# etri/bwa-mem-scale

Hardware: AMD Instinct MI355X
Metric: Mreads/sec through the GPU hot path (seed -> chain -> extend -> dedup, reads and index resident), 150bp SE vs a synthetic genome of GRCh38 size, at 1 MI355X; % HBM roofline in roofline.frac (higher is better)
Workload: dtype int64 intervals / int16 DP (two columns per register; int32 for queries beyond 191 bases or scores beyond 2^14)

## Files before the change

bwa-mem-scale_amd/bwams/capi.py:

```python
from __future__ import annotations

import ctypes as C
import os
import subprocess

import numpy as np

PKG = os.path.dirname(os.path.dirname(os.path.abspath(__file__)))
LIB_PATH = os.environ.get("BWAMS_LIB") or os.path.join(PKG, "_build", "libbwams.so")

SMEM_DTYPE = np.dtype([("rid", "<u4"), ("m", "<u4"), ("n", "<u4"), ("pad_", "<u4"),
                       ("k", "<i8"), ("l", "<i8"), ("s", "<i8")])
SEQPAIR_DTYPE = np.dtype([(n, "<i4") for n in
                          ("idr", "idq", "id", "len1", "len2", "h0", "seqid", "regid",
                           "score", "tle", "gtle", "qle", "gscore", "max_off")])

SYMBOLS = [
    "bwams_strerror", "bwams_last_error", "bwams_device_count", "bwams_debug_reload",
    "bwams_index_open", "bwams_index_from_host", "bwams_index_from_device", "bwams_index_close",
    "bwams_index_bytes", "bwams_index_build", "bwams_index_fetch", "bwams_index_save", "bwams_reg2aln_run", "bwams_reg2aln_run_sam", "bwams_reg2aln_fetch",
    "bwams_index_set_contig_names", "bwams_index_set_contig_annos", "bwams_sam_upload", "bwams_sam_run", "bwams_sam_run_pe", "bwams_sam_run_emf", "bwams_sam_fetch",
    "bwams_process_chunk", "bwams_process_chunk_smart", "bwams_process_chunk2", "bwams_emf_regs_merge", "bwams_fastq_decode", "bwams_fastq_info", "bwams_fastq_has_qual", "bwams_fastq_fetch", "bwams_fastq_to_batch", "bwams_fastq_to_batch_opt", "bwams_fastq_close", "bwams_batch_create", "bwams_batch_destroy", "bwams_seed_fmi",
    "bwams_seed_upload", "bwams_seed_run", "bwams_seed_counts", "bwams_seed_fetch",
    "bwams_ert_from_host", "bwams_ert_open", "bwams_ert_close", "bwams_ert_bytes", "bwams_ert_set_fat", "bwams_seed_run_ert",
    "bwams_ert_build", "bwams_ert_info", "bwams_ert_fetch", "bwams_ert_save", "bwams_debug_sort", "bwams_debug_regs_upload", "bwams_debug_aln_lists",
    "bwams_debug_ext_regs_upload", "bwams_debug_dedup_counts", "bwams_debug_pair_regs_upload", "bwams_debug_pair_counts", "bwams_debug_chain_counts", "bwams_debug_chain_lane_counts",
    "bwams_emf_build", "bwams_emf_info", "bwams_emf_table_fetch", "bwams_emf_save",
    "bwams_bsw_extend", "bwams_bsw_upload", "bwams_bsw_run", "bwams_bsw_fetch",
    "bwams_batch_stats", "bwams_batch_sync", "bwams_ksw_align",
    "bwams_index_build_fma", "bwams_index_set_fma", "bwams_index_fetch_fma",
    "bwams_index_from_fasta", "bwams_index_from_fasta_file", "bwams_index_load_bns",
    "bwams_emf_open", "bwams_emf_from_host", "bwams_emf_close", "bwams_emf_probe",
    "bwams_emf_from_device", "bwams_emf_run", "bwams_emf_fetch",
    "bwams_index_set_contigs", "bwams_chain_run", "bwams_chain_fetch", "bwams_chain_upload",
# ... 1297 lines not shown
        L.bwams_reg2aln_run.argtypes = [vp, vp, i32, vp, vp, vp]
        L.bwams_reg2aln_fetch.argtypes = [vp, vp, i64, vp, i64, vp, i64]
        L.bwams_debug_regs_upload.argtypes = [vp, vp, i64, vp, i64]
        L.bwams_debug_aln_lists.argtypes = [vp, vp]
        L.bwams_debug_ext_regs_upload.argtypes = [vp, vp, i64, vp, i64]
        L.bwams_debug_dedup_counts.argtypes = [vp, vp]
        L.bwams_debug_pair_regs_upload.argtypes = [vp, vp, i64, vp, i64]
        L.bwams_debug_pair_counts.argtypes = [vp, vp]
        L.bwams_debug_chain_counts.argtypes = [vp, vp]
        L.bwams_debug_chain_lane_counts.argtypes = [vp, vp]
        L.bwams_index_build_fma.argtypes = [vp, C.c_int, C.c_int]
        L.bwams_index_set_fma.argtypes = [vp, vp, C.c_int, vp, C.c_int]
        L.bwams_index_fetch_fma.argtypes = [vp, vp, vp]
        L.bwams_index_bytes.restype = i64
        L.bwams_index_bytes.argtypes = [vp]
        L.bwams_batch_create.argtypes = [vp, i64, i64, i64, i64, vp]
        L.bwams_batch_destroy.argtypes = [vp]
        L.bwams_seed_fmi.argtypes = [vp, vp, vp, vp, i64, vp, vp, i64, vp, vp, i64, vp, vp]
        L.bwams_seed_upload.argtypes = [vp, vp, vp, vp, i64]
        L.bwams_index_set_contigs.argtypes = [vp, vp, i32]
        L.bwams_chain_run.argtypes = [vp, vp, vp, vp]
        L.bwams_chain_fetch.argtypes = [vp, vp, i64, vp, i64, vp]
        L.bwams_chain_upload.argtypes = [vp, vp, i64, vp, i64, vp]
        L.bwams_extend_build.argtypes = [vp, vp, vp, vp]
        L.bwams_extend_run.argtypes = [vp, vp, vp]
        L.bwams_extend_fetch.argtypes = [vp, vp, i64, vp, vp]
        L.bwams_extend_tasks_fetch.argtypes = [vp, i32, vp, i64, vp, i64, vp, i64, vp, vp, vp]
        L.bwams_dedup_run.argtypes = [vp, vp, vp]
        L.bwams_dedup_fetch.argtypes = [vp, vp, i64, vp]
        L.bwams_pestat.argtypes = [vp, vp, vp]
# ... 199 lines not shown
            blob += (a if isinstance(a, bytes) else a.encode()) + b"\0"
        off.append(len(blob))
        off = np.asarray(off, np.int32)
        _chk(lib().bwams_index_set_contig_annos(self.h, bytes(blob), _p(off)), "bwams_index_set_contig_annos")

    def debug_sort(self, k, s, q, which: int, mode: int = 0):
        k = np.ascontiguousarray(k, np.int64); s = np.ascontiguousarray(s, np.int32); q = np.ascontiguousarray(q, np.int32)
        out = np.zeros(len(k), np.int32)
        _chk(lib().bwams_debug_sort(self.h, _p(k), _p(s), _p(q), len(k), which, mode, _p(out)), "bwams_debug_sort")
        return out

    @property
    def nbytes(self) -> int:
        return lib().bwams_index_bytes(self.h)

    def close(self):
        if self.h:
            lib().bwams_index_close(self.h)
            self.h = None


class Emf:

    def __init__(self, index: Index, table=None, path: str | None = None, device_table=None):
        self.index = index
        self.h = C.c_void_p()
        self._keep = device_table
        if device_table is not None:
            t = device_table
            _chk(lib().bwams_emf_from_device(index.h, t.seed_len, t.seq_len, t.loc_table.data_ptr(), t.loc_table.numel(),
                                             t.seed_table.data_ptr(), t.seed_table.shape[0], C.byref(self.h)),
                 "bwams_emf_from_device")
        elif path is not None:
            _chk(lib().bwams_emf_open(index.h, path.encode(), C.byref(self.h)), "bwams_emf_open")
# ... 921 lines not shown
```

bwa-mem-scale_amd/csrc/api.hip:

```cpp
#include <fcntl.h>
#include <sys/mman.h>
#include <sys/stat.h>
#include <unistd.h>

#include <algorithm>
#include <cstring>

#include "stage_state.h"

namespace bwams {

static Knobs g_knobs;
static std::once_flag g_knobs_once;
static int env_int(const char *name, int dflt) { const char *e = getenv(name); return e && *e ? atoi(e) : dflt; }
void knobs_reload() {
    Knobs k;
    { const char *vb = getenv("BWAMS_VERBOSE"); k.verbose = vb && *vb && *vb != '0'; }
    k.debug = env_int("BWAMS_DEBUG", 0);
    k.poison = env_int("BWAMS_POISON", 0);
    k.bwd_min_list = env_int("BWAMS_BWD_MIN_LIST", k.bwd_min_list); k.bwd_cols = env_int("BWAMS_BWD_COLS", k.bwd_cols);
    k.bwd_late_list = env_int("BWAMS_BWD_LATE_LIST", k.bwd_late_list);
    k.bwd_dry_min_list = env_int("BWAMS_BWD_DRY_MIN_LIST", k.bwd_dry_min_list); k.bwd_dry_cols = env_int("BWAMS_BWD_DRY_COLS", k.bwd_dry_cols);
    k.bwd_dry_late_list = env_int("BWAMS_BWD_DRY_LATE_LIST", k.bwd_dry_late_list);
    k.r3_beside = env_int("BWAMS_SEED_R3_BESIDE", 1);
    k.ext_max_rounds = env_int("BWAMS_EXT_MAX_ROUNDS", 0); k.ext_all_rounds = getenv("BWAMS_EXT_ALL_ROUNDS") != nullptr;
    k.ext_inplace = env_int("BWAMS_EXT_INPLACE", 1);
    k.dedup_seq = env_int("BWAMS_DEDUP_SEQ", 0) == 1;
    k.dedup_count = env_int("BWAMS_DEDUP_COUNT", 0) == 1;
    k.pair_count = env_int("BWAMS_PAIR_COUNT", 0) == 1;
    k.pair_drop_plan = getenv("BWAMS_PAIR_DROP_PLAN") != nullptr;
    k.trace_pair = env_int("BWAMS_TRACE_PAIR", 0);
    k.bsw_pk = env_int("BWAMS_BSW_PK", 1);
    k.chain_batch = env_int("BWAMS_CHAIN_BATCH", 1);
    k.chain_count = env_int("BWAMS_CHAIN_COUNT", 0) == 1;
    k.depth_combine = env_int("BWAMS_DEPTH_COMBINE", 1);
    k.pileup_tiled = env_int("BWAMS_PILEUP_TILED", 1);
    k.qc_lanes = env_int("BWAMS_QC_LANES", 1);
    k.recal_lds = env_int("BWAMS_RECAL_LDS", 1);
    k.ert_ticket = env_int("BWAMS_ERT_TICKET", 1); k.ert_grid = env_int("BWAMS_ERT_GRID", -1); k.ert_fat = env_int("BWAMS_ERT_FAT", 1);
    g_knobs = k;
}
const Knobs &knobs() {
    std::call_once(g_knobs_once, knobs_reload);
    return g_knobs;
}

static thread_local std::string g_last_error;
void set_last_error(const std::string &s) { g_last_error = s; }

int check_device(int device) {
    int n = 0;
    hipError_t e = hipGetDeviceCount(&n);
    if (e != hipSuccess || n <= 0) {
        set_last_error(std::string("no HIP device: ") + hipGetErrorString(e));
// ... 205 lines not shown
```

bwa-mem-scale_amd/csrc/api_index.hip:

```cpp
#include <cstring>

#include "fmi_kernels.h"

namespace bwams {
int fmi_build_device(bwams_index *ix, const uint8_t *d_fw, int64_t l_pac, int keep_ref, int64_t chunk_rows, int verbose,
                     bwams_build_stats_t *bs);
}

using namespace bwams;

extern "C" {

static int index_finish(bwams_index *ix, const bwams_fmi_desc_t *d, const void *cp, const void *ms, const void *ls, const void *ref) {
    ix->fmi.cp = reinterpret_cast<const uint4 *>(cp);
    ix->fmi.cp2 = nullptr;
    ix->fmi.sa_ms = reinterpret_cast<const int8_t *>(ms);
    ix->fmi.sa_ls = reinterpret_cast<const uint32_t *>(ls);
    ix->fmi.ref = reinterpret_cast<const uint8_t *>(ref);
    if (d->ref_seq_len >= ((int64_t)1 << 36)) {
        set_last_error("text longer than 2^36 rows is not supported by the 36-bit interval packing");
        return BWAMS_ERR_UNSUPPORTED;
    }
    for (int i = 0; i < 5; ++i) ix->fmi.count[i] = d->count[i];
    ix->fmi.sentinel = d->sentinel_index;
// ... 174 lines not shown
    if (rc == BWAMS_ERR_IO) set_last_error("write failed: " + path);
    if (!rc && ix->bns) rc = bns_save(ix, prefix);
    return rc;
}

int bwams_index_close(bwams_index_t *ix) {
    if (!ix) return BWAMS_OK;
    (void)hipSetDevice(ix->device);
    delete ix->bns;
    delete ix;
    return BWAMS_OK;
}

int64_t bwams_index_bytes(const bwams_index_t *ix) { return ix ? ix->bytes : 0; }


static int fma_alloc(bwams_index *ix, int all_bp, int last_bp) {
    if (all_bp < 2 || all_bp > 11 || last_bp < 2 || last_bp > 13) {
        set_last_error("FMA depths must be 2..11 (all_smem) and 2..13 (last_smem)");
        return BWAMS_ERR_ARG;
    }
    BWAMS_HIP(hipSetDevice(ix->device));
    ix->d_all.release();
    ix->d_last.release();
    ix->fmi.all_smem = nullptr;
    ix->fmi.last_smem = nullptr;
    BWAMS_HIP(ix->d_all.alloc(((size_t)1 << (2 * all_bp)) * 128));
    BWAMS_HIP(ix->d_last.alloc(((size_t)1 << (2 * last_bp)) * 16));
    return BWAMS_OK;
}
// ... 44 lines not shown
```

bwa-mem-scale_amd/csrc/api_seed.hip:

```cpp
#include <algorithm>
#include <cstring>
#include <mutex>

#include <rocprim/rocprim.hpp>

#include "fmi_kernels.h"
#include "ert_kernels.h"
#include "stage_state.h"

namespace bwams {

int alloc_smem_buffers(bwams_batch *b, int64_t max_smem) {
    b->sd.d_pool.release(); b->sd.d_sorted.release(); b->sd.d_keys.release(); b->sd.d_keys2.release(); b->sd.d_vals.release();
    b->sd.d_vals2.release(); b->sd.d_work2.release(); b->sd.d_sa_off.release(); b->sd.d_sa_cnt.release();
    b->max_smem = max_smem;
    b->pool_cap = b->max_smem + seed_pool_slack(b->cu_count);
    BWAMS_HIP(b->sd.d_pool.alloc((size_t)b->pool_cap * sizeof(bwams_smem_t)));
    BWAMS_HIP(b->sd.d_sorted.alloc((size_t)b->max_smem * sizeof(bwams_smem_t)));
    BWAMS_HIP(b->sd.d_keys.alloc((size_t)b->pool_cap * 8));
    BWAMS_HIP(b->sd.d_keys2.alloc((size_t)b->pool_cap * 8));
    BWAMS_HIP(b->sd.d_vals.alloc((size_t)b->pool_cap * 4));
    BWAMS_HIP(b->sd.d_vals2.alloc((size_t)b->pool_cap * 4));
    BWAMS_HIP(b->sd.d_work2.alloc((size_t)b->pool_cap * sizeof(Round2Work)));
    BWAMS_HIP(b->sd.d_sa_off.alloc((size_t)(b->max_smem + 1) * 8));
// ... 4 lines not shown
int alloc_seed_tmp(bwams_batch *b) {
    size_t t1 = 0, t2 = 0;
    (void)rocprim::radix_sort_pairs(nullptr, t1, b->sd.d_keys.p, b->sd.d_keys2.p, b->sd.d_vals.p, b->sd.d_vals2.p,
                              (size_t)b->max_smem, 0, 64, b->stream);
    (void)rocprim::exclusive_scan(nullptr, t2, b->sd.d_sa_cnt.p, b->sd.d_sa_off.p, (int64_t)0, (size_t)b->max_smem + 1,
                            rocprim::plus<int64_t>(), b->stream);
    BWAMS_HIP(b->d_tmp.alloc(std::max(t1, t2)));
    return BWAMS_OK;
}

namespace {

int sort_pool(bwams_batch *b, const char *who, int64_t n_keys, int64_t n, int64_t *sa_cnt, int max_occ) {
    bwams_batch::Seed &sd = b->sd;
    hipStream_t st = b->stream;
    launch_make_keys(sd.d_pool.p, n_keys, sd.d_keys.p, sd.d_vals.p, (uint32_t)b->nseq, st);
    int rid_bits = 1;
    while (((int64_t)1 << rid_bits) <= b->nseq) rid_bits++;
    if (int rc = with_tmp(b, who, [&](void *tmp, size_t &tb) {
            return rocprim::radix_sort_pairs(tmp, tb, sd.d_keys.p, sd.d_keys2.p, sd.d_vals.p, sd.d_vals2.p, (size_t)n_keys, 0, 32 + rid_bits, st);
        })) return rc;
    launch_gather_sorted(sd.d_pool.p, sd.d_vals2.p, n, sd.d_sorted.p, sa_cnt, max_occ, st);
    return BWAMS_OK;
}

void fm_lookup(bwams_batch *b, int64_t n) {
    bwams_batch::Seed &sd = b->sd;
    launch_sa_lookup(b->idx->fmi, sd.d_sorted.p, n, sd.d_sa_off.p, sd.d_sa_coord.p, b->max_sa, sd.last_opt.max_occ, b->d_ctr.p, b->cu_count, b->stream);
}
void ert_locate(bwams_batch *b, int64_t n) {
    bwams_batch::Seed &sd = b->sd;
    launch_ert_locate(sd.ert->t, b->d_enc.p, b->d_cum.p, sd.d_sorted.p, n, sd.with_sa ? sd.d_sa_cnt.p : nullptr, sd.last_opt.max_occ, b->d_ctr.p,
                      sd.d_ert_stk.p, sd.ert_stk_frames, b->cu_count, b->stream);
}
int ert_gather(bwams_batch *b, int64_t n) {
    bwams_batch::Seed &sd = b->sd;
    const int64_t cap = n + n / 4 + 1024;
    BWAMS_HIP(sd.d_ert_redo.ensure((size_t)((n + 31) / 32) * 4, (size_t)((cap + 31) / 32) * 4));
    launch_ert_gather(sd.ert->t, sd.d_sorted.p, n, sd.d_sa_off.p, sd.d_sa_coord.p, b->max_sa, sd.last_opt.max_occ, b->d_ctr.p, sd.d_ert_stk.p,
                      sd.ert_stk_frames, sd.d_ert_redo.p, b->max_sa, b->cu_count, b->stream);
    return BWAMS_OK;
}

// ... 86 lines not shown
    b->sd.n_smem = b->sd.n_sa = 0;

    const uint4 *cp2 = nullptr;
    {
        bwams_index *ix = b->idx;
        std::lock_guard<std::mutex> lock(ix->cp2_mu);
        if (!ix->d_cp2.p) {
            DevBuf<> t;
            BWAMS_HIP(t.alloc(cp2_bytes(ix->n_blk)));
            launch_cp2_build(ix->fmi.cp, ix->n_blk, t.as<uint4>(), st);
            BWAMS_HIP(hipStreamSynchronize(st));
            ix->d_cp2 = std::move(t);
        }
        cp2 = ix->d_cp2.as<const uint4>();
    }
    SeedLaunch a;
    a.fmi = b->idx->fmi;
    a.fmi.cp2 = cp2;
    a.enc = b->d_enc.p;
    a.cum = b->d_cum.p;
    a.skip = b->has_skip ? b->d_skip.p : nullptr;
    a.nseq = b->nseq;
    a.packed = b->sd.d_packed.p;
    a.read_w = b->sd.read_w;
    a.read_cw = b->sd.read_cw;
    a.reads_in_lds = b->sd.read_w <= 40;
    a.debug = knobs().debug;
    a.min_seed_len = opt->min_seed_len;
    a.pool = b->sd.d_pool.p;
    a.pool_cap = b->pool_cap;
// ... 277 lines not shown
```

bwa-mem-scale_amd/csrc/common.h:

```cpp
#pragma once

#include <cstdlib>
#include <hip/hip_runtime.h>
#include <mutex>
#include <stdint.h>
#include <stdio.h>
#include <string>
#include <vector>

#include "../../include/bwams.h"
#include "stage_valid.h"

namespace bwams {

void set_last_error(const std::string &s);

struct Knobs {
    int verbose = 0;
    int debug = 0;
    int poison = 0;
    int bwd_min_list = 40, bwd_cols = 24, bwd_late_list = 8;
    int bwd_dry_min_list = 24, bwd_dry_cols = 8, bwd_dry_late_list = 12;
    int r3_beside = 1;
    int ext_max_rounds = 0;
    int ext_all_rounds = 0;
    int ext_inplace = 1;
    int dedup_seq = 0;
    int dedup_count = 0;
    int pair_count = 0;
    int pair_drop_plan = 0;
    int trace_pair = 0;
    int bsw_pk = 1;
    int chain_count = 0;
    int chain_batch = 1;
    int ert_fat = 1;
    int depth_combine = 1;
    int pileup_tiled = 1;
    int qc_lanes = 1;
    int recal_lds = 1;
    int ert_grid = -1, ert_ticket = 1;
};
const Knobs &knobs();
void knobs_reload();

template <class T> static inline hipError_t dev_malloc(T **p, size_t bytes) {
    const bool poison = knobs().poison != 0;
    hipError_t e = hipMalloc(reinterpret_cast<void **>(p), bytes);
    if (e == hipSuccess && poison && bytes) {
        e = hipMemset(*p, 0xAB, bytes);
        if (e == hipSuccess) e = hipDeviceSynchronize();
    }
    return e;
}

template <class T = void, bool Host = false> struct Buf {
    T *p = nullptr;
    size_t cap = 0;
    Buf() = default;
    Buf(Buf &&o) noexcept : p(o.p), cap(o.cap) { o.p = nullptr; o.cap = 0; }
    Buf &operator=(Buf &&o) noexcept {
        if (this != &o) { release(); p = o.p; cap = o.cap; o.p = nullptr; o.cap = 0; }
        return *this;
    }
    ~Buf() { release(); }
    template <class U> U *as() const { return reinterpret_cast<U *>(p); }
    void release() {
        if (p) (void)(Host ? hipHostFree(p) : hipFree(p));
        p = nullptr;
        cap = 0;
    }
    hipError_t alloc(size_t bytes) {
        release();
        hipError_t e = Host ? hipHostMalloc(&p, bytes, hipHostMallocDefault) : dev_malloc(&p, bytes);
        cap = p ? bytes : 0;
        return e;
    }
    hipError_t ensure(size_t bytes, size_t new_cap) { return bytes <= cap ? hipSuccess : alloc(new_cap); }
    hipError_t ensure(size_t bytes) { return ensure(bytes, bytes + bytes / 8 + 4096); }
    hipError_t ensure_n(size_t n) { return ensure(n * sizeof(T)); }
};
template <class T = void> using DevBuf = Buf<T, false>;
template <class T = void> using HostBuf = Buf<T, true>;

#define BWAMS_HIP(call)                                                                  \
    do {                                                                                 \
        hipError_t e_ = (call);                                                          \
        if (e_ != hipSuccess) {                                                          \
            char buf_[512];                                                              \
// ... 539 lines not shown
};
namespace bwams {
int fastq_classify(bwams_fastq *f, std::vector<uint8_t> *which);
int fastq_subset(bwams_fastq *f, const std::vector<int64_t> &ids, bwams_fastq **out);
int fastq_interleave(bwams_fastq *f1, bwams_fastq *f2, bwams_fastq **out);
}

struct bwams_index {
    int device = 0;
    bwams::DevFmi fmi{};
    int64_t bytes = 0;
    int64_t n_blk = 0, n_sa = 0;
    bwams::DevBuf<> d_cp, d_ms, d_ls, d_ref;
    bwams::DevBuf<> d_cp2;
    std::mutex cp2_mu;
    bwams::DevBuf<> d_all, d_last;
    bwams::DevBuf<> d_contigs;
    int32_t n_seqs = 0;
    bwams::DevBuf<> d_ctg_annos, d_ctg_anno_off;
    bwams::DevBuf<> d_ctg_names, d_ctg_off;
    bwams::BnsMeta *bns = nullptr;
    std::vector<std::string> h_ctg_names;
    bwams::DevBuf<> d_ctg_sorted;
    bool ctg_dup = false;
};

namespace bwams {
int bns_save(bwams_index *ix, const char *prefix);
int bam_names_index(bwams_index *ix, const char *names, const int32_t *name_off, int32_t n);
}

struct bwams_ert {
    bwams_index *idx = nullptr;
    bwams::DevErt t{};
    bwams::DevBuf<> d_kmer, d_mlt, d_cnt, d_fat;
    int64_t bytes = 0, mlt_bytes = 0, n_big = 0;
    float build_ms[3] = {0, 0, 0};
};

struct bwams_emf {
    bwams_index *idx = nullptr;
    bwams::DevEmf t{};
    bwams::DevBuf<> d_seeds, d_loc;
// ... 129 lines not shown
```

bwa-mem-scale_amd/csrc/fmi_kernels.h:

```cpp
#pragma once
#include "common.h"

namespace bwams {

struct SeedLaunch {
    DevFmi fmi;
    const uint8_t *enc;
    const int64_t *cum;
    const uint8_t *skip;
    const uint32_t *packed;
    int read_w, read_cw;
    int reads_in_lds;
    int debug;
    int64_t nseq;
    int min_seed_len;
    bwams_smem_t *pool;
    int64_t pool_cap;
    DevCounters *ctr;
    uint4 *prev;
    int prev_cap;
    int64_t prev_threads;
    BwdItem *bwd_items, *bwd_items_s;
    uint4 *bwd_ent;
    int64_t bwd_items_cap, bwd_ent_cap;
// ... 7 lines not shown
int64_t seed_pool_slack(int cu_count);

void launch_pack_reads(const uint8_t *enc, const int64_t *cum, int64_t nseq, int W, int cw, uint32_t *packed,
                       hipStream_t st);
void launch_mark(DevCounters *ctr, int which, hipStream_t st);
void launch_smem_round1(const SeedLaunch &a, int cu_count, hipStream_t st);
void launch_round2_work(const SeedLaunch &a, Round2Work *work, int64_t work_cap, int split_len,
                        int split_width, int cu_count, hipStream_t st);
void launch_smem_round2(const SeedLaunch &a, const Round2Work *work, int cu_count, hipStream_t st);
void launch_smem_bwd_wave(const SeedLaunch &a, int cu_count, hipStream_t st);
void launch_smem_round3(const SeedLaunch &a, int max_intv, int cu_count, hipStream_t st);

void launch_build_fma(const DevFmi &f, int all_bp, uint32_t *all_tab, int last_bp, uint4 *last_tab, hipStream_t st);

void launch_make_keys(const bwams_smem_t *pool, int64_t n, uint64_t *keys, uint32_t *vals, uint32_t hole_key_rid,
                      hipStream_t st);
void launch_gather_sorted(const bwams_smem_t *pool, const uint32_t *order, int64_t n, bwams_smem_t *sorted,
                          int64_t *sa_cnt, int max_occ, hipStream_t st);
void launch_sa_lookup(const DevFmi &f, const bwams_smem_t *sorted, int64_t n_smem, const int64_t *sa_off,
                      int64_t *coord, int64_t coord_cap, int max_occ, DevCounters *ctr, int cu_count,
                      hipStream_t st);

size_t cp2_bytes(int64_t n_blk);
void launch_cp2_build(const uint4 *cp, int64_t n_blk, uint4 *cp2, hipStream_t st);

}
```

bwa-mem-scale_amd/csrc/fmi_sal.hip:

```cpp
#include "fmi_kernels.h"

namespace bwams {
namespace {

__device__ __forceinline__ uint64_t mk64(uint32_t lo, uint32_t hi) {
    return (uint64_t)lo | ((uint64_t)hi << 32);
}

__global__ __launch_bounds__(256) void sa_lookup_kernel(DevFmi f, const bwams_smem_t *__restrict__ sm,
                                                        int64_t n_smem, const int64_t *__restrict__ sa_off,
                                                        int64_t *__restrict__ coord, int64_t coord_cap,
                                                        int max_occ, DevCounters *ctr) {
    const int64_t total = sa_off[n_smem] < coord_cap ? sa_off[n_smem] : coord_cap;
    unsigned long long lf = 0;
    __shared__ int64_t win_s[4][65];
    int64_t *const win = win_s[threadIdx.x >> 6];
    const int lane = (int)(threadIdx.x & 63);
    const int64_t n_waves = (int64_t)gridDim.x * 4, wave = (int64_t)blockIdx.x * 4 + (threadIdx.x >> 6);
    const int64_t per = ((total + n_waves - 1) / n_waves + 63) & ~(int64_t)63;
    const int64_t start = wave * per, end = start + per < total ? start + per : total;
    int64_t lo0 = 0;
    if (start < end) {
        int64_t a = 0, b = n_smem;
        while (b - a > 1) {
            const int64_t mid = (a + b) >> 1;
            if (sa_off[mid] <= start) a = mid; else b = mid;
        }
// ... 19 lines not shown
                const int64_t mid = (a + b) >> 1;
                if (sa_off[mid] <= g) a = mid; else b = mid;
            }
            lo = a;
        }
        {
            const int last = (int)((end - g0 < 64 ? end - g0 : 64) - 1);
            const uint32_t l_lo = (uint32_t)lo, l_hi = (uint32_t)((uint64_t)lo >> 32);
            lo0 = (int64_t)(((uint64_t)(uint32_t)__builtin_amdgcn_readlane((int)l_hi, last) << 32) | (uint32_t)__builtin_amdgcn_readlane((int)l_lo, last));
        }
        __builtin_amdgcn_wave_barrier();
        if (g >= end) continue;
        const int64_t k = sm[lo].k, s = sm[lo].s;
        const int64_t step = s > (int64_t)max_occ ? s / max_occ : 1;
        int64_t sp = k + (g - sa_off[lo]) * step;
        int64_t off = 0, val = 0;
        while (true) {
            if ((sp & 7) == 0) {
                val = ((int64_t)f.sa_ms[sp >> 3] << 32) + (int64_t)f.sa_ls[sp >> 3] + off;
                break;
            }
            const uint4 *p = f.cp + ((sp >> 6) << 2);
            const uint4 c01 = p[0], c23 = p[1], h01 = p[2], h23 = p[3];
            const int sh = 63 - (int)(sp & 63);
            const uint64_t h0 = mk64(h01.x, h01.y), h1 = mk64(h01.z, h01.w);
            const uint64_t h2 = mk64(h23.x, h23.y), h3 = mk64(h23.z, h23.w);
            int b = 4;
            uint64_t hb = 0;
            if ((h0 >> sh) & 1) { b = 0; hb = h0; }
            else if ((h1 >> sh) & 1) { b = 1; hb = h1; }
            else if ((h2 >> sh) & 1) { b = 2; hb = h2; }
            else if ((h3 >> sh) & 1) { b = 3; hb = h3; }
            if (b == 4) { val = 0; break; }
            const int y = (int)(sp & 63);
            const uint64_t mask = y ? (~0ull << (64 - y)) : 0ull;
            const int64_t cnt = (int64_t)(b == 0 ? mk64(c01.x, c01.y) : b == 1 ? mk64(c01.z, c01.w) : b == 2 ? mk64(c23.x, c23.y) : mk64(c23.z, c23.w));
            sp = (b == 0 ? f.count[0] : b == 1 ? f.count[1] : b == 2 ? f.count[2] : f.count[3]) + cnt +
                 __popcll(hb & mask);
            off++;
            lf++;
        }
        coord[g] = val;
    }
    for (int o = 32; o > 0; o >>= 1)
        lf += mk64(__shfl_down((uint32_t)lf, o), __shfl_down((uint32_t)(lf >> 32), o));
    if ((threadIdx.x & 63) == 0 && lf) atomicAdd(&ctr->n_lf_steps, lf);
    if (blockIdx.x == 0 && threadIdx.x == 0) ctr->n_sa_lookups = (unsigned long long)sa_off[n_smem];
}

}

void launch_sa_lookup(const DevFmi &f, const bwams_smem_t *sorted, int64_t n_smem, const int64_t *sa_off,
                      int64_t *coord, int64_t coord_cap, int max_occ, DevCounters *ctr, int cu_count,
                      hipStream_t st) {
    if (n_smem <= 0) return;
    sa_lookup_kernel<<<cu_count * 8, 256, 0, st>>>(f, sorted, n_smem, sa_off, coord, coord_cap, max_occ, ctr);
}

}
```

bwa-mem-scale_amd/csrc/fmi_seed.hip:

```cpp
#include "fmi_kernels.h"
#include "wave_ops.h"

namespace bwams {

namespace {

constexpr int kBlock = 256;
constexpr int kBlocksPerCU = 6;

__device__ __forceinline__ uint64_t mk64(uint32_t lo, uint32_t hi) {
    return (uint64_t)lo | ((uint64_t)hi << 32);
}

struct Occ4 {
    int64_t v[4];
};

template <int CTRL>
__device__ __forceinline__ uint32_t qdpp(uint32_t v) {
    return (uint32_t)__builtin_amdgcn_update_dpp(0, (int)v, CTRL, 0xF, 0xF, false);
}

__device__ __forceinline__ void occ_from_block(const uint4 &c01, const uint4 &c23, const uint4 &h01,
                                               const uint4 &h23, int64_t pos, Occ4 &o) {
// ... 1246 lines not shown
                em_n = (uint32_t)j;
                em_k = ck; em_l = cl; em_s = cs;
                x = next_x;
                phase = PH_PIVOT;
            }
            j++;
        }
        if (phase == PH_HOLD) phase = PH_FWD;
        wave_emit(a, wo, em, rid, em_m, em_n, em_k, em_l, em_s);
    }
    wave_emit_finish(a, wo, true);
    flush_counters(a.ctr, n_ext, n_blk, true);
}

__global__ void make_keys_kernel(const bwams_smem_t *pool, int64_t n, uint64_t *keys, uint32_t *vals,
                                 uint32_t hole_key_rid) {
    const int64_t i = (int64_t)blockIdx.x * blockDim.x + threadIdx.x;
    if (i < n) {
        const bwams_smem_t s = pool[i];
        const uint32_t rid = s.rid == kHoleRid ? hole_key_rid : s.rid;
        keys[i] = ((uint64_t)rid << 32) | ((uint64_t)(s.m & 0xffff) << 16) | (uint64_t)(s.n & 0xffff);
        vals[i] = (uint32_t)i;
    }
}

__global__ void gather_sorted_kernel(const bwams_smem_t *pool, const uint32_t *order, int64_t n,
                                     bwams_smem_t *sorted, int64_t *sa_cnt, int max_occ) {
    const int64_t i = (int64_t)blockIdx.x * blockDim.x + threadIdx.x;
    if (i < n) {
        const bwams_smem_t s = pool[order[i]];
        sorted[i] = s;
        if (sa_cnt) sa_cnt[i] = s.s < (int64_t)max_occ ? s.s : (int64_t)max_occ;
    }
}

__global__ void cpi_build_kernel(const uint4 *__restrict__ cp, int64_t n_blk, uint4 *__restrict__ out) {
// ... 60 lines not shown
void launch_smem_round2(const SeedLaunch &a, const Round2Work *work, int cu_count, hipStream_t st) {
    smem_search_kernel<false><<<grid_for(a.nseq, cu_count), kBlock, lds_bytes_search(a), st>>>(a, work);
}

void launch_smem_bwd_wave(const SeedLaunch &a, int cu_count, hipStream_t st) {
    if (a.bwd_min_list <= 0) return;
    const size_t lds = (size_t)(kBlock / 64) * (kBwdMaxList * 16 + 16 * (size_t)(a.read_w <= kBwdReadLds ? a.read_w : 0));
    smem_bwd_kernel<<<cu_count * 8, kBlock, lds, st>>>(a);
}

void launch_smem_round3(const SeedLaunch &a, int max_intv, int cu_count, hipStream_t st) {
    seed_strategy_kernel<<<grid_for(a.nseq, cu_count), kBlock, lds_bytes(a), st>>>(a, max_intv);
}

void launch_make_keys(const bwams_smem_t *pool, int64_t n, uint64_t *keys, uint32_t *vals, uint32_t hole_key_rid,
                      hipStream_t st) {
    if (n <= 0) return;
    make_keys_kernel<<<(unsigned)((n + 255) / 256), 256, 0, st>>>(pool, n, keys, vals, hole_key_rid);
}

void launch_gather_sorted(const bwams_smem_t *pool, const uint32_t *order, int64_t n, bwams_smem_t *sorted,
                          int64_t *sa_cnt, int max_occ, hipStream_t st) {
    if (n <= 0) return;
    gather_sorted_kernel<<<(unsigned)((n + 255) / 256), 256, 0, st>>>(pool, order, n, sorted, sa_cnt, max_occ);
}

}
```

include/bwams.h:

```cpp
#ifndef BWAMS_H
#define BWAMS_H

#include <stddef.h>
#include <stdint.h>
#include "bwams_types.h"

#ifdef __cplusplus
extern "C" {
#endif

#define BWAMS_OK               0
#define BWAMS_ERR_DEVICE      -1
#define BWAMS_ERR_IO          -2
#define BWAMS_ERR_ARG         -3
#define BWAMS_ERR_CAPACITY    -4
#define BWAMS_ERR_NOMEM       -5
#define BWAMS_ERR_UNSUPPORTED -6

typedef struct bwams_index bwams_index_t;
typedef struct bwams_batch bwams_batch_t;
typedef struct bwams_emf bwams_emf_t;

const char *bwams_strerror(int code);
const char *bwams_last_error(void);
// ... 69 lines not shown
typedef struct bwams_deflater bwams_deflater_t;
typedef struct bwams_deflate_stats {
    int64_t members, in_bytes, out_bytes;
    float ms_upload, ms_kernel, ms_download;
} bwams_deflate_stats_t;
#define BWAMS_DEFLATE_EOF 0x1
int64_t bwams_deflate_bound(int64_t n_bytes);
int bwams_deflater_create(int device, int64_t max_in_bytes, bwams_deflater_t **out);
int bwams_deflater_run(bwams_deflater_t *d, const void *in, int64_t n_bytes, int in_on_device, void *out, int64_t out_cap,
                       int out_on_device, int32_t flags, int64_t *n_out, bwams_deflate_stats_t *stats);
int bwams_deflater_destroy(bwams_deflater_t *d);
int bwams_index_load_bns(bwams_index_t *idx, const char *prefix);

int bwams_index_close(bwams_index_t *idx);
int64_t bwams_index_bytes(const bwams_index_t *idx);


int bwams_batch_create(bwams_index_t *idx, int64_t max_reads, int64_t max_bases,
                       int64_t max_smem, int64_t max_sa, bwams_batch_t **out);
int bwams_batch_destroy(bwams_batch_t *b);


int bwams_seed_fmi(bwams_batch_t *b,
                   const uint8_t *enc_qdb, const int64_t *cum_len, const uint8_t *skip,
                   int64_t nseq, const bwams_seed_opt_t *opt,
                   bwams_smem_t *smem_out, int64_t smem_cap, int64_t *n_smem,
                   int64_t *sa_coord, int64_t sa_cap, int64_t *sa_off, int64_t *n_sa);

int bwams_seed_upload(bwams_batch_t *b, const uint8_t *enc_qdb, const int64_t *cum_len,
                      const uint8_t *skip, int64_t nseq);
// ... 411 lines not shown
```

Baseline: 11.25.

## Add lazily built dense suffix-array table and narrow seed sort keys

Builds a full-resolution (stride 1 by default) suffix-array coordinate table on the device the first time seeding with SA lookup runs. sa_lookup then does one indexed load instead of walking the BWT up to seven LF steps per hit to reach a sampled SA entry. The table is about 8 bytes per reference position (tens of GB for a GRCh38-sized genome). It can be refused under a byte cap or released when another allocation runs out of memory. Separately, seed sort keys use 8-bit position fields when reads are at most 255 bases, cutting radix sort passes.

```diff
diff --git a/bwa-mem-scale_amd/bwams/capi.py b/bwa-mem-scale_amd/bwams/capi.py
--- a/bwa-mem-scale_amd/bwams/capi.py
+++ b/bwa-mem-scale_amd/bwams/capi.py
@@ -18,6 +18,7 @@
 SYMBOLS = [
     "bwams_strerror", "bwams_last_error", "bwams_device_count", "bwams_debug_reload",
     "bwams_index_open", "bwams_index_from_host", "bwams_index_from_device", "bwams_index_close",
+    "bwams_debug_sa_dense_state", "bwams_debug_sa_dense_fetch", "bwams_debug_sa_dense_release",
     "bwams_index_bytes", "bwams_index_build", "bwams_index_fetch", "bwams_index_save", "bwams_reg2aln_run", "bwams_reg2aln_run_sam", "bwams_reg2aln_fetch",
     "bwams_index_set_contig_names", "bwams_index_set_contig_annos", "bwams_sam_upload", "bwams_sam_run", "bwams_sam_run_pe", "bwams_sam_run_emf", "bwams_sam_fetch",
     "bwams_process_chunk", "bwams_process_chunk_smart", "bwams_process_chunk2", "bwams_emf_regs_merge", "bwams_fastq_decode", "bwams_fastq_info", "bwams_fastq_has_qual", "bwams_fastq_fetch", "bwams_fastq_to_batch", "bwams_fastq_to_batch_opt", "bwams_fastq_close", "bwams_batch_create", "bwams_batch_destroy", "bwams_seed_fmi",
@@ -1345,6 +1346,9 @@
         L.bwams_index_fetch_fma.argtypes = [vp, vp, vp]
         L.bwams_index_bytes.restype = i64
         L.bwams_index_bytes.argtypes = [vp]
+        L.bwams_debug_sa_dense_state.argtypes = [vp, vp, vp, vp, vp]
+        L.bwams_debug_sa_dense_fetch.argtypes = [vp, vp, i64, vp]
+        L.bwams_debug_sa_dense_release.argtypes = [C.c_int, vp]
         L.bwams_batch_create.argtypes = [vp, i64, i64, i64, i64, vp]
         L.bwams_batch_destroy.argtypes = [vp]
         L.bwams_seed_fmi.argtypes = [vp, vp, vp, vp, i64, vp, vp, i64, vp, vp, i64, vp, vp]
@@ -1574,10 +1578,31 @@
     def nbytes(self) -> int:
         return lib().bwams_index_bytes(self.h)
 
+    def sa_dense_state(self):
+        st, sr, nb, ms = C.c_int32(0), C.c_int32(0), C.c_int64(0), C.c_float(0)
+        _chk(lib().bwams_debug_sa_dense_state(self.h, C.byref(st), C.byref(sr), C.byref(nb), C.byref(ms)), "bwams_debug_sa_dense_state")
+        return SA_DENSE_STATES[st.value], sr.value, nb.value, ms.value
+
+    def sa_dense_fetch(self) -> np.ndarray:
+        n = C.c_int64(0)
+        _chk(lib().bwams_debug_sa_dense_fetch(self.h, None, 0, C.byref(n)), "bwams_debug_sa_dense_fetch")
+        out = np.zeros(n.value, np.uint64)
+        _chk(lib().bwams_debug_sa_dense_fetch(self.h, _p(out), len(out), C.byref(n)), "bwams_debug_sa_dense_fetch")
+        return out
+
     def close(self):
         if self.h:
             lib().bwams_index_close(self.h)
             self.h = None
+
+
+SA_DENSE_STATES = ("absent", "built", "refused", "yielded")
+
+
+def sa_dense_release(device: int = 0) -> int:
+    n = C.c_int32(0)
+    _chk(lib().bwams_debug_sa_dense_release(device, C.byref(n)), "bwams_debug_sa_dense_release")
+    return n.value
 
 
 class Emf:
diff --git a/bwa-mem-scale_amd/csrc/api.hip b/bwa-mem-scale_amd/csrc/api.hip
--- a/bwa-mem-scale_amd/csrc/api.hip
+++ b/bwa-mem-scale_amd/csrc/api.hip
@@ -38,6 +38,10 @@
     k.qc_lanes = env_int("BWAMS_QC_LANES", 1);
     k.recal_lds = env_int("BWAMS_RECAL_LDS", 1);
     k.ert_ticket = env_int("BWAMS_ERT_TICKET", 1); k.ert_grid = env_int("BWAMS_ERT_GRID", -1); k.ert_fat = env_int("BWAMS_ERT_FAT", 1);
+    k.sa_dense = env_int("BWAMS_SA_DENSE", kSaDenseDefault);
+    if (k.sa_dense != 0 && k.sa_dense != 1 && k.sa_dense != 2 && k.sa_dense != 4) k.sa_dense = kSaDenseDefault;
+    { const char *mb = getenv("BWAMS_SA_DENSE_MAX_BYTES"); k.sa_dense_max_bytes = mb && *mb ? atoll(mb) : 0; }
+    k.sort_narrow = env_int("BWAMS_SORT_NARROW", 1);
     g_knobs = k;
 }
 const Knobs &knobs() {
diff --git a/bwa-mem-scale_amd/csrc/api_index.hip b/bwa-mem-scale_amd/csrc/api_index.hip
--- a/bwa-mem-scale_amd/csrc/api_index.hip
+++ b/bwa-mem-scale_amd/csrc/api_index.hip
@@ -5,6 +5,94 @@
 namespace bwams {
 int fmi_build_device(bwams_index *ix, const uint8_t *d_fw, int64_t l_pac, int keep_ref, int64_t chunk_rows, int verbose,
                      bwams_build_stats_t *bs);
+
+static std::mutex g_ix_mu;
+static std::vector<bwams_index *> g_ix;
+}
+
+bwams_index::bwams_index() {
+    std::lock_guard<std::mutex> reg(bwams::g_ix_mu);
+    bwams::g_ix.push_back(this);
+}
+bwams_index::~bwams_index() {
+    std::lock_guard<std::mutex> reg(bwams::g_ix_mu);
+    for (size_t i = 0; i < bwams::g_ix.size(); ++i)
+        if (bwams::g_ix[i] == this) { bwams::g_ix.erase(bwams::g_ix.begin() + i); break; }
+}
+
+namespace bwams {
+
+int sa_dense_release(int device) {
+    int n = 0;
+    std::lock_guard<std::mutex> reg(g_ix_mu);
+    for (bwams_index *ix : g_ix) {
+        if (ix->device != device) continue;
+        std::unique_lock<std::shared_mutex> lock(ix->sa_mu);
+        if (ix->sa_state != BWAMS_SA_DENSE_BUILT) continue;
+        (void)hipDeviceSynchronize();
+        ix->d_sa_dense.release();
+        ix->sa_bytes = 0;
+        ix->sa_state = BWAMS_SA_DENSE_YIELDED;
+        if (knobs().verbose) fprintf(stderr, "[sa_dense] device %d out of memory: the table of stride %d gave way\n", device, ix->sa_stride);
+        ++n;
+    }
+    return n;
+}
+
+int sa_dense_ensure(bwams_index *ix, int cu_count, hipStream_t st) {
+    const Knobs &kn = knobs();
+    if (kn.sa_dense == 0) return BWAMS_OK;
+    {
+        std::shared_lock<std::shared_mutex> lock(ix->sa_mu);
+        if (ix->sa_state != BWAMS_SA_DENSE_ABSENT) return BWAMS_OK;
+    }
+    std::unique_lock<std::shared_mutex> lock(ix->sa_mu);
+    if (ix->sa_state != BWAMS_SA_DENSE_ABSENT) return BWAMS_OK;
+    const int stride = kn.sa_dense;
+    const int64_t n = sa_dense_entries(ix->fmi.ref_seq_len, stride), bytes = n * 8;
+    ix->sa_stride = stride;
+    if (kn.sa_dense_max_bytes > 0 && bytes > kn.sa_dense_max_bytes) {
+        ix->sa_state = BWAMS_SA_DENSE_REFUSED;
+        return BWAMS_OK;
+    }
+    DevBuf<> t;
+    if (t.alloc((size_t)bytes + 8, false) != hipSuccess) {
+        (void)hipGetLastError();
+        ix->sa_state = BWAMS_SA_DENSE_REFUSED;
+        if (kn.verbose) fprintf(stderr, "[sa_dense] no room for %.1f GiB: the index keeps the walk\n", bytes / 1073741824.0);
+        return BWAMS_OK;
+    }
+    unsigned long long *d_bad = reinterpret_cast<unsigned long long *>(t.as<uint64_t>() + n), bad = 0;
+    hipEvent_t ev[2];
+    BWAMS_HIP(hipEventCreate(&ev[0]));
+    BWAMS_HIP(hipEventCreate(&ev[1]));
+    hipError_t e = hipMemsetAsync(d_bad, 0, 8, st);
+    if (e == hipSuccess) e = hipEventRecord(ev[0], st);
+    if (e == hipSuccess) {
+        launch_sa_dense_build(ix->fmi, stride, n, t.as<uint64_t>(), d_bad, cu_count, st);
+        e = hipGetLastError();
+    }
+    if (e == hipSuccess) e = hipEventRecord(ev[1], st);
+    if (e == hipSuccess) e = hipMemcpyAsync(&bad, d_bad, 8, hipMemcpyDeviceToHost, st);
+    if (e == hipSuccess) e = hipStreamSynchronize(st);
+    float ms = 0;
+    if (e == hipSuccess) e = hipEventElapsedTime(&ms, ev[0], ev[1]);
+    (void)hipEventDestroy(ev[0]);
+    (void)hipEventDestroy(ev[1]);
+    BWAMS_HIP(e);
+    ix->sa_build_ms = ms;
+    if (bad) {
+        fprintf(stderr, "[sa_dense] a walk of this index does not fit the table's %d-bit step field: the index keeps the walk\n", kSaDenseStepBits);
+        ix->sa_state = BWAMS_SA_DENSE_REFUSED;
+        return BWAMS_OK;
+    }
+    ix->d_sa_dense = std::move(t);
+    ix->sa_bytes = bytes;
+    ix->sa_state = BWAMS_SA_DENSE_BUILT;
+    if (kn.verbose) fprintf(stderr, "[sa_dense] stride %d: %lld entries, %.2f GiB, built in %.1f ms\n", stride, (long long)n, bytes / 1073741824.0, ms);
+    return BWAMS_OK;
+}
+
 }
 
 using namespace bwams;
@@ -212,6 +300,40 @@
 
 int64_t bwams_index_bytes(const bwams_index_t *ix) { return ix ? ix->bytes : 0; }
 
+int bwams_debug_sa_dense_state(bwams_index_t *ix, int32_t *state, int32_t *stride, int64_t *bytes, float *build_ms) {
+    if (!ix) return BWAMS_ERR_ARG;
+    std::shared_lock<std::shared_mutex> lock(ix->sa_mu);
+    if (state) *state = ix->sa_state;
+    if (stride) *stride = ix->sa_stride;
+    if (bytes) *bytes = ix->sa_bytes.load();
+    if (build_ms) *build_ms = ix->sa_build_ms;
+    return BWAMS_OK;
+}
+
+int bwams_debug_sa_dense_fetch(bwams_index_t *ix, uint64_t *out, int64_t cap, int64_t *n) {
+    if (!ix || !n) return BWAMS_ERR_ARG;
+    BWAMS_HIP(hipSetDevice(ix->device));
+    std::shared_lock<std::shared_mutex> lock(ix->sa_mu);
+    if (ix->sa_state != BWAMS_SA_DENSE_BUILT) {
+        set_last_error("bwams_debug_sa_dense_fetch: the index holds no dense table");
+        return BWAMS_ERR_ARG;
+    }
+    *n = sa_dense_entries(ix->fmi.ref_seq_len, ix->sa_stride);
+    if (!out) return BWAMS_OK;
+    if (cap < *n) return BWAMS_ERR_CAPACITY;
+    BWAMS_HIP(hipMemcpy(out, ix->d_sa_dense.p, (size_t)*n * 8, hipMemcpyDeviceToHost));
+    return BWAMS_OK;
+}
+
+int bwams_debug_sa_dense_release(int device, int32_t *n_released) {
+    int rc = check_device(device);
+    if (rc) return rc;
+    BWAMS_HIP(hipSetDevice(device));
+    const int n = sa_dense_release(device);
+    if (n_released) *n_released = n;
+    return BWAMS_OK;
+}
+
 
 static int fma_alloc(bwams_index *ix, int all_bp, int last_bp) {
     if (all_bp < 2 || all_bp > 11 || last_bp < 2 || last_bp > 13) {
diff --git a/bwa-mem-scale_amd/csrc/api_seed.hip b/bwa-mem-scale_amd/csrc/api_seed.hip
--- a/bwa-mem-scale_amd/csrc/api_seed.hip
+++ b/bwa-mem-scale_amd/csrc/api_seed.hip
@@ -42,11 +42,12 @@
 int sort_pool(bwams_batch *b, const char *who, int64_t n_keys, int64_t n, int64_t *sa_cnt, int max_occ) {
     bwams_batch::Seed &sd = b->sd;
     hipStream_t st = b->stream;
-    launch_make_keys(sd.d_pool.p, n_keys, sd.d_keys.p, sd.d_vals.p, (uint32_t)b->nseq, st);
+    const int w = b->max_read_len <= 255 && knobs().sort_narrow ? 8 : 16;
+    launch_make_keys(sd.d_pool.p, n_keys, sd.d_keys.p, sd.d_vals.p, (uint32_t)b->nseq, w, st);
     int rid_bits = 1;
     while (((int64_t)1 << rid_bits) <= b->nseq) rid_bits++;
     if (int rc = with_tmp(b, who, [&](void *tmp, size_t &tb) {
-            return rocprim::radix_sort_pairs(tmp, tb, sd.d_keys.p, sd.d_keys2.p, sd.d_vals.p, sd.d_vals2.p, (size_t)n_keys, 0, 32 + rid_bits, st);
+            return rocprim::radix_sort_pairs(tmp, tb, sd.d_keys.p, sd.d_keys2.p, sd.d_vals.p, sd.d_vals2.p, (size_t)n_keys, 0, 2 * w + rid_bits, st);
         })) return rc;
     launch_gather_sorted(sd.d_pool.p, sd.d_vals2.p, n, sd.d_sorted.p, sa_cnt, max_occ, st);
     return BWAMS_OK;
@@ -54,7 +55,11 @@
 
 void fm_lookup(bwams_batch *b, int64_t n) {
     bwams_batch::Seed &sd = b->sd;
-    launch_sa_lookup(b->idx->fmi, sd.d_sorted.p, n, sd.d_sa_off.p, sd.d_sa_coord.p, b->max_sa, sd.last_opt.max_occ, b->d_ctr.p, b->cu_count, b->stream);
+    bwams_index *ix = b->idx;
+    std::shared_lock<std::shared_mutex> lock(ix->sa_mu);
+    const bool use = ix->sa_state == BWAMS_SA_DENSE_BUILT && knobs().sa_dense != 0;
+    launch_sa_lookup(ix->fmi, sd.d_sorted.p, n, sd.d_sa_off.p, sd.d_sa_coord.p, b->max_sa, sd.last_opt.max_occ, b->d_ctr.p, b->cu_count, b->stream,
+                     use ? ix->d_sa_dense.as<const uint64_t>() : nullptr, ix->sa_stride);
 }
 void ert_locate(bwams_batch *b, int64_t n) {
     bwams_batch::Seed &sd = b->sd;
@@ -171,6 +176,8 @@
         }
         cp2 = ix->d_cp2.as<const uint4>();
     }
+    if (with_sa)
+        if (int rc = sa_dense_ensure(b->idx, b->cu_count, st)) return rc;
     SeedLaunch a;
     a.fmi = b->idx->fmi;
     a.fmi.cp2 = cp2;
diff --git a/bwa-mem-scale_amd/csrc/common.h b/bwa-mem-scale_amd/csrc/common.h
--- a/bwa-mem-scale_amd/csrc/common.h
+++ b/bwa-mem-scale_amd/csrc/common.h
@@ -1,8 +1,10 @@
 #pragma once
 
+#include <atomic>
 #include <cstdlib>
 #include <hip/hip_runtime.h>
 #include <mutex>
+#include <shared_mutex>
 #include <stdint.h>
 #include <stdio.h>
 #include <string>
@@ -15,6 +17,7 @@
 
 void set_last_error(const std::string &s);
 
+constexpr int kSaDenseDefault = 1;
 struct Knobs {
     int verbose = 0;
     int debug = 0;
@@ -39,13 +42,23 @@
     int qc_lanes = 1;
     int recal_lds = 1;
     int ert_grid = -1, ert_ticket = 1;
+    int sa_dense = kSaDenseDefault;
+    int64_t sa_dense_max_bytes = 0;
+    int sort_narrow = 1;
 };
 const Knobs &knobs();
 void knobs_reload();
 
-template <class T> static inline hipError_t dev_malloc(T **p, size_t bytes) {
+int sa_dense_release(int device);
+
+template <class T> static inline hipError_t dev_malloc(T **p, size_t bytes, bool may_yield = true) {
     const bool poison = knobs().poison != 0;
     hipError_t e = hipMalloc(reinterpret_cast<void **>(p), bytes);
+    if (e == hipErrorOutOfMemory && may_yield) {
+        int dev = 0;
+        (void)hipGetLastError();
+        if (hipGetDevice(&dev) == hipSuccess && sa_dense_release(dev) > 0) e = hipMalloc(reinterpret_cast<void **>(p), bytes);
+    }
     if (e == hipSuccess && poison && bytes) {
         e = hipMemset(*p, 0xAB, bytes);
         if (e == hipSuccess) e = hipDeviceSynchronize();
@@ -69,9 +82,9 @@
         p = nullptr;
         cap = 0;
     }
-    hipError_t alloc(size_t bytes) {
+    hipError_t alloc(size_t bytes, bool may_yield = true) {
         release();
-        hipError_t e = Host ? hipHostMalloc(&p, bytes, hipHostMallocDefault) : dev_malloc(&p, bytes);
+        hipError_t e = Host ? hipHostMalloc(&p, bytes, hipHostMallocDefault) : dev_malloc(&p, bytes, may_yield);
         cap = p ? bytes : 0;
         return e;
     }
@@ -641,6 +654,13 @@
     bwams::DevBuf<> d_cp, d_ms, d_ls, d_ref;
     bwams::DevBuf<> d_cp2;
     std::mutex cp2_mu;
+    bwams::DevBuf<> d_sa_dense;
+    std::shared_mutex sa_mu;
+    int sa_state = BWAMS_SA_DENSE_ABSENT, sa_stride = 0;
+    float sa_build_ms = 0;
+    std::atomic<int64_t> sa_bytes{0};
+    bwams_index();
+    ~bwams_index();
     bwams::DevBuf<> d_all, d_last;
     bwams::DevBuf<> d_contigs;
     int32_t n_seqs = 0;
@@ -654,6 +674,7 @@
 
 namespace bwams {
 int bns_save(bwams_index *ix, const char *prefix);
+int sa_dense_ensure(bwams_index *ix, int cu_count, hipStream_t st);
 int bam_names_index(bwams_index *ix, const char *names, const int32_t *name_off, int32_t n);
 }
 
diff --git a/bwa-mem-scale_amd/csrc/fmi_kernels.h b/bwa-mem-scale_amd/csrc/fmi_kernels.h
--- a/bwa-mem-scale_amd/csrc/fmi_kernels.h
+++ b/bwa-mem-scale_amd/csrc/fmi_kernels.h
@@ -45,12 +45,52 @@
 void launch_build_fma(const DevFmi &f, int all_bp, uint32_t *all_tab, int last_bp, uint4 *last_tab, hipStream_t st);
 
 void launch_make_keys(const bwams_smem_t *pool, int64_t n, uint64_t *keys, uint32_t *vals, uint32_t hole_key_rid,
-                      hipStream_t st);
+                      int pos_bits, hipStream_t st);
 void launch_gather_sorted(const bwams_smem_t *pool, const uint32_t *order, int64_t n, bwams_smem_t *sorted,
                           int64_t *sa_cnt, int max_occ, hipStream_t st);
 void launch_sa_lookup(const DevFmi &f, const bwams_smem_t *sorted, int64_t n_smem, const int64_t *sa_off,
                       int64_t *coord, int64_t coord_cap, int max_occ, DevCounters *ctr, int cu_count,
-                      hipStream_t st);
+                      hipStream_t st, const uint64_t *dense = nullptr, int stride = 0);
+
+constexpr int kSaDenseCoordBits = 40, kSaDenseStepBits = 23;
+constexpr uint64_t kSaDenseSentinel = 1ull << kSaDenseCoordBits;
+inline int64_t sa_dense_entries(int64_t rows, int stride) { return (rows + stride - 1) / stride; }
+void launch_sa_dense_build(const DevFmi &f, int stride, int64_t n, uint64_t *table, unsigned long long *bad, int cu_count, hipStream_t st);
+
+#ifdef __HIPCC__
+struct SaWalk {
+    int64_t sp;
+    uint32_t steps;
+    bool sentinel;
+};
+template <int S> __device__ __forceinline__ SaWalk sa_walk(const DevFmi &f, int64_t sp) {
+    auto mk64 = [](uint32_t lo, uint32_t hi) { return (uint64_t)lo | ((uint64_t)hi << 32); };
+    SaWalk w{sp, 0, false};
+    while ((w.sp & (S - 1)) != 0) {
+        const uint4 *p = f.cp + ((w.sp >> 6) << 2);
+        const uint4 c01 = p[0], c23 = p[1], h01 = p[2], h23 = p[3];
+        const int sh = 63 - (int)(w.sp & 63);
+        const uint64_t h0 = mk64(h01.x, h01.y), h1 = mk64(h01.z, h01.w);
+        const uint64_t h2 = mk64(h23.x, h23.y), h3 = mk64(h23.z, h23.w);
+        int b = 4;
+        uint64_t hb = 0;
+        if ((h0 >> sh) & 1) { b = 0; hb = h0; }
+        else if ((h1 >> sh) & 1) { b = 1; hb = h1; }
+        else if ((h2 >> sh) & 1) { b = 2; hb = h2; }
+        else if ((h3 >> sh) & 1) { b = 3; hb = h3; }
+        if (b == 4) { w.sentinel = true; break; }
+        const int y = (int)(w.sp & 63);
+        const uint64_t mask = y ? (~0ull << (64 - y)) : 0ull;
+        const int64_t cnt = (int64_t)(b == 0 ? mk64(c01.x, c01.y) : b == 1 ? mk64(c01.z, c01.w) : b == 2 ? mk64(c23.x, c23.y) : mk64(c23.z, c23.w));
+        w.sp = (b == 0 ? f.count[0] : b == 1 ? f.count[1] : b == 2 ? f.count[2] : f.count[3]) + cnt + __popcll(hb & mask);
+        w.steps++;
+    }
+    return w;
+}
+__device__ __forceinline__ int64_t sa_sample(const DevFmi &f, int64_t sp) {
+    return ((int64_t)f.sa_ms[sp >> 3] << 32) + (int64_t)f.sa_ls[sp >> 3];
+}
+#endif
 
 size_t cp2_bytes(int64_t n_blk);
 void launch_cp2_build(const uint4 *cp, int64_t n_blk, uint4 *cp2, hipStream_t st);
diff --git a/bwa-mem-scale_amd/csrc/fmi_sal.hip b/bwa-mem-scale_amd/csrc/fmi_sal.hip
--- a/bwa-mem-scale_amd/csrc/fmi_sal.hip
+++ b/bwa-mem-scale_amd/csrc/fmi_sal.hip
@@ -7,10 +7,11 @@
     return (uint64_t)lo | ((uint64_t)hi << 32);
 }
 
+template <int S>
 __global__ __launch_bounds__(256) void sa_lookup_kernel(DevFmi f, const bwams_smem_t *__restrict__ sm,
                                                         int64_t n_smem, const int64_t *__restrict__ sa_off,
                                                         int64_t *__restrict__ coord, int64_t coord_cap,
-                                                        int max_occ, DevCounters *ctr) {
+                                                        int max_occ, DevCounters *ctr, const uint64_t *__restrict__ dense) {
     const int64_t total = sa_off[n_smem] < coord_cap ? sa_off[n_smem] : coord_cap;
     unsigned long long lf = 0;
     __shared__ int64_t win_s[4][65];
@@ -60,31 +61,20 @@
         const int64_t k = sm[lo].k, s = sm[lo].s;
         const int64_t step = s > (int64_t)max_occ ? s / max_occ : 1;
         int64_t sp = k + (g - sa_off[lo]) * step;
-        int64_t off = 0, val = 0;
-        while (true) {
-            if ((sp & 7) == 0) {
-                val = ((int64_t)f.sa_ms[sp >> 3] << 32) + (int64_t)f.sa_ls[sp >> 3] + off;
-                break;
+        int64_t val;
+        if constexpr (S == 0) {
+            const SaWalk w = sa_walk<8>(f, sp);
+            val = w.sentinel ? 0 : sa_sample(f, w.sp) + (int64_t)w.steps;
+            lf += w.steps;
+        } else {
+            const SaWalk w = sa_walk<S>(f, sp);
+            uint64_t e = kSaDenseSentinel;
+            if (!w.sentinel) {
+                e = dense[S == 1 ? w.sp : S == 2 ? w.sp >> 1 : w.sp >> 2];
+                lf += e >> (kSaDenseCoordBits + 1);
             }
-            const uint4 *p = f.cp + ((sp >> 6) << 2);
-            const uint4 c01 = p[0], c23 = p[1], h01 = p[2], h23 = p[3];
-            const int sh = 63 - (int)(sp & 63);
-            const uint64_t h0 = mk64(h01.x, h01.y), h1 = mk64(h01.z, h01.w);
-            const uint64_t h2 = mk64(h23.x, h23.y), h3 = mk64(h23.z, h23.w);
-            int b = 4;
-            uint64_t hb = 0;
-            if ((h0 >> sh) & 1) { b = 0; hb = h0; }
-            else if ((h1 >> sh) & 1) { b = 1; hb = h1; }
-            else if ((h2 >> sh) & 1) { b = 2; hb = h2; }
-            else if ((h3 >> sh) & 1) { b = 3; hb = h3; }
-            if (b == 4) { val = 0; break; }
-            const int y = (int)(sp & 63);
-            const uint64_t mask = y ? (~0ull << (64 - y)) : 0ull;
-            const int64_t cnt = (int64_t)(b == 0 ? mk64(c01.x, c01.y) : b == 1 ? mk64(c01.z, c01.w) : b == 2 ? mk64(c23.x, c23.y) : mk64(c23.z, c23.w));
-            sp = (b == 0 ? f.count[0] : b == 1 ? f.count[1] : b == 2 ? f.count[2] : f.count[3]) + cnt +
-                 __popcll(hb & mask);
-            off++;
-            lf++;
+            val = (e & kSaDenseSentinel) ? 0 : (int64_t)(e & (kSaDenseSentinel - 1)) + (int64_t)w.steps;
+            lf += w.steps;
         }
         coord[g] = val;
     }
@@ -94,13 +84,33 @@
     if (blockIdx.x == 0 && threadIdx.x == 0) ctr->n_sa_lookups = (unsigned long long)sa_off[n_smem];
 }
 
+__global__ __launch_bounds__(256) void sa_dense_build_kernel(DevFmi f, int stride, int64_t n, uint64_t *__restrict__ table,
+                                                             unsigned long long *bad) {
+    for (int64_t i = (int64_t)blockIdx.x * 256 + threadIdx.x; i < n; i += (int64_t)gridDim.x * 256) {
+        const SaWalk w = sa_walk<8>(f, i * stride);
+        if (w.steps >> kSaDenseStepBits) *bad = 1;
+        const uint64_t c = w.sentinel ? kSaDenseSentinel : (uint64_t)(sa_sample(f, w.sp) + (int64_t)w.steps);
+        if (!w.sentinel && (c >> kSaDenseCoordBits)) *bad = 1;
+        table[i] = c | ((uint64_t)w.steps << (kSaDenseCoordBits + 1));
+    }
+}
+
 }
 
 void launch_sa_lookup(const DevFmi &f, const bwams_smem_t *sorted, int64_t n_smem, const int64_t *sa_off,
                       int64_t *coord, int64_t coord_cap, int max_occ, DevCounters *ctr, int cu_count,
-                      hipStream_t st) {
+                      hipStream_t st, const uint64_t *dense, int stride) {
     if (n_smem <= 0) return;
-    sa_lookup_kernel<<<cu_count * 8, 256, 0, st>>>(f, sorted, n_smem, sa_off, coord, coord_cap, max_occ, ctr);
+    const unsigned grid = (unsigned)cu_count * 8;
+    if (!dense) sa_lookup_kernel<0><<<grid, 256, 0, st>>>(f, sorted, n_smem, sa_off, coord, coord_cap, max_occ, ctr, nullptr);
+    else if (stride == 1) sa_lookup_kernel<1><<<grid, 256, 0, st>>>(f, sorted, n_smem, sa_off, coord, coord_cap, max_occ, ctr, dense);
+    else if (stride == 2) sa_lookup_kernel<2><<<grid, 256, 0, st>>>(f, sorted, n_smem, sa_off, coord, coord_cap, max_occ, ctr, dense);
+    else sa_lookup_kernel<4><<<grid, 256, 0, st>>>(f, sorted, n_smem, sa_off, coord, coord_cap, max_occ, ctr, dense);
+}
+
+void launch_sa_dense_build(const DevFmi &f, int stride, int64_t n, uint64_t *table, unsigned long long *bad, int cu_count, hipStream_t st) {
+    if (n <= 0) return;
+    sa_dense_build_kernel<<<grid_of(n, 256, cu_count, 32), 256, 0, st>>>(f, stride, n, table, bad);
 }
 
 }
diff --git a/bwa-mem-scale_amd/csrc/fmi_seed.hip b/bwa-mem-scale_amd/csrc/fmi_seed.hip
--- a/bwa-mem-scale_amd/csrc/fmi_seed.hip
+++ b/bwa-mem-scale_amd/csrc/fmi_seed.hip
@@ -1284,12 +1284,13 @@
 }
 
 __global__ void make_keys_kernel(const bwams_smem_t *pool, int64_t n, uint64_t *keys, uint32_t *vals,
-                                 uint32_t hole_key_rid) {
+                                 uint32_t hole_key_rid, int pos_bits) {
     const int64_t i = (int64_t)blockIdx.x * blockDim.x + threadIdx.x;
     if (i < n) {
         const bwams_smem_t s = pool[i];
         const uint32_t rid = s.rid == kHoleRid ? hole_key_rid : s.rid;
-        keys[i] = ((uint64_t)rid << 32) | ((uint64_t)(s.m & 0xffff) << 16) | (uint64_t)(s.n & 0xffff);
+        const uint32_t mask = (1u << pos_bits) - 1;
+        keys[i] = ((uint64_t)rid << (2 * pos_bits)) | ((uint64_t)(s.m & mask) << pos_bits) | (uint64_t)(s.n & mask);
         vals[i] = (uint32_t)i;
     }
 }
@@ -1380,9 +1381,9 @@
 }
 
 void launch_make_keys(const bwams_smem_t *pool, int64_t n, uint64_t *keys, uint32_t *vals, uint32_t hole_key_rid,
-                      hipStream_t st) {
+                      int pos_bits, hipStream_t st) {
     if (n <= 0) return;
-    make_keys_kernel<<<(unsigned)((n + 255) / 256), 256, 0, st>>>(pool, n, keys, vals, hole_key_rid);
+    make_keys_kernel<<<(unsigned)((n + 255) / 256), 256, 0, st>>>(pool, n, keys, vals, hole_key_rid, pos_bits);
 }
 
 void launch_gather_sorted(const bwams_smem_t *pool, const uint32_t *order, int64_t n, bwams_smem_t *sorted,
diff --git a/include/bwams.h b/include/bwams.h
--- a/include/bwams.h
+++ b/include/bwams.h
@@ -107,6 +107,14 @@
 
 int bwams_index_close(bwams_index_t *idx);
 int64_t bwams_index_bytes(const bwams_index_t *idx);
+
+enum { BWAMS_SA_DENSE_ABSENT = 0,
+       BWAMS_SA_DENSE_BUILT = 1,
+       BWAMS_SA_DENSE_REFUSED = 2,
+       BWAMS_SA_DENSE_YIELDED = 3 };
+int bwams_debug_sa_dense_state(bwams_index_t *idx, int32_t *state, int32_t *stride, int64_t *bytes, float *build_ms);
+int bwams_debug_sa_dense_fetch(bwams_index_t *idx, uint64_t *out, int64_t cap, int64_t *n);
+int bwams_debug_sa_dense_release(int device, int32_t *n_released);
 
 
 int bwams_batch_create(bwams_index_t *idx, int64_t max_reads, int64_t max_bases,
```

After: 11.78, median of 6. +4.7%, better.
